# medvedevgroup/SibeliaZ

Measured on AMD Instinct MI355X. Metric: seed vertices/sec through BlocksFinder, higher is better.
Workload: dtype int32

## Files before the change

sibeliaz_amd/csrc/lcb_kernel.h:

```cpp
#ifndef LCB_KERNEL_H
#define LCB_KERNEL_H

#include <hip/hip_runtime.h>
#include <stdint.h>

#include "lcb_kernel_limits.h"

#define LCB_EMPTY_KEY INT32_MIN
#if defined(__HIP_DEVICE_COMPILE__)
#define LCB_NO_LOADS_IN_FLIGHT() __builtin_amdgcn_s_waitcnt(0x0F70)
#else
#define LCB_NO_LOADS_IN_FLIGHT() ((void)0)
#endif
#if defined(__HIP_DEVICE_COMPILE__)
#define LCB_GLOBAL_U32(p) ((const __attribute__((address_space(1))) uint32_t*)(p))
#else
#define LCB_GLOBAL_U32(p) (p)
#endif
#ifndef LCB_PROF_PUSH
#define LCB_PROF_PUSH 0
#endif

template <int MODE> struct LcbCfg;
template <> struct LcbCfg<0> { static constexpr uint32_t IC = 256, VC = 1024, BW = 256, PC = 0; static constexpr bool INST_LDS = true, IDX_LDS = true, WINDOW_WALK = true, RESOLVE = false; typedef uint16_t Idx; typedef uint32_t VLast; };
// ... 186 lines not shown
    uint8_t* fpSeg8;
    uint32_t* fpSeg32;
    uint32_t nFp;
    uint32_t fpSplit, fpShift;
    uint32_t instCap;
    int32_t* vKey;
    uint32_t* vCount;
    VLast* vLast;
    Idx* vTouched;
    uint32_t* vNClaimed;
    uint32_t* vTicket;
    uint32_t* vOvf;
    uint32_t* vRec;
    uint32_t* vItem;
    uint32_t voteCap, voteShift;
    uint32_t* scr;
    uint32_t* bloom;
    uint32_t bloomShift;
    uint32_t* mail;
    uint32_t* part;
    unsigned long long* mailWalk;
    int32_t* pKeys;
    uint32_t* pSlots;
    uint32_t pathCap, pathShift;
    unsigned long long* body;
    uint32_t bodyCap;
    uint4* best;
    uint32_t bestCap;
    uint32_t* ck;
    uint32_t ckN, ckInst, ckGood, ckPath;
    int32_t ckFlank;
    uint32_t nInst, nGood, cur, nPath, nRight, nLeft, nBest, status;
    int32_t rightFlank, leftFlank;
    uint32_t* dbg;
    const uint32_t* abort;
    uint32_t pfPush, pfVote, pfMaxProbe, pfMaxInst;
    uint64_t pfTVote, pfTPush, pfTScore;
    uint64_t pfTWalk, pfTWaitB, pfTReduce, pfTScan;
    uint64_t pfVoters, pfChunks, pfTouchSum;
    uint64_t cWalk, cOcc, cCompatCall, cCompatStep, cVote, cPush;
};

#ifndef LCB_TEST_FP_SLOT_DIV
#define LCB_TEST_FP_SLOT_DIV 1u
#endif
template <class ST>
__device__ __forceinline__ uint32_t lcb_fp_slot(const ST& S, uint32_t i)
{
    if (i < S.fpSplit) return i;
    const uint32_t f = i + S.fpShift;
    return f < S.instCap / LCB_TEST_FP_SLOT_DIV ? f : i;
}

template <class ST>
__device__ __forceinline__ void lcb_fp_set_seg(ST& S, uint32_t fs, uint32_t seg)
{
    if (ST::SEG) { if (LcbCfg<ST::MODE>::INST_LDS) S.fpSeg8[fs] = (uint8_t)seg; else S.fpSeg32[fs] = seg; }
}
template <class ST>
__device__ __forceinline__ uint32_t lcb_fp_get_seg(const ST& S, uint32_t fs)
{
    return ST::SEG ? (LcbCfg<ST::MODE>::INST_LDS ? (uint32_t)S.fpSeg8[fs] : S.fpSeg32[fs]) : 0u;
}

enum { LCB_F_FRONTG = 0, LCB_F_BACKG, LCB_F_FRONTPOS, LCB_F_BACKPOS, LCB_F_LO, LCB_F_HI, LCB_F_FLAGS, LCB_F_FRONTDIST, LCB_F_BACKDIST, LCB_F_COUNT };
template <class ST>
// ... 58 lines not shown
    const uint32_t wa = (uint32_t)(a >> 5), wb = (uint32_t)((b - 1) >> 5);
    const uint32_t ma = 0xFFFFFFFFu << ((uint32_t)a & 31), mb = 0xFFFFFFFFu >> (31 - ((uint32_t)(b - 1) & 31));
    if (wa == wb) return (lcb_uword(U, wa) & ma & mb) != 0;
    if (lcb_uword(U, wa) & ma) return true;
    for (uint32_t w = wa + 1; w < wb; w++)
        if (lcb_uword(U, w)) return true;
    return (lcb_uword(U, wb) & mb) != 0;
}

template <class F>
__device__ inline uint32_t lcb_range_walk_steps(const LcbUsed& used, F a, F b, bool up)
{
    uint32_t steps = 0;
    if (up) { for (F g = a; g < b; g++) { steps++; if (lcb_used_bit(used, g)) break; } }
    else { for (F g = b; g > a; g--) { steps++; if (lcb_used_bit(used, (F)(g - 1))) break; } }
    return steps;
}

__device__ __forceinline__ uint32_t lcb_bcast(uint32_t v, uint32_t src) { return (uint32_t)__shfl((int)v, (int)src); }

#define LCB_DPP_ADD64(v, ctrl, rowMask)                                                                             \
    do {                                                                                                            \
        const uint32_t lo_ = (uint32_t)__builtin_amdgcn_update_dpp(0, (int)(uint32_t)(v), ctrl, rowMask, 0xf, false); \
        const uint32_t hi_ = (uint32_t)__builtin_amdgcn_update_dpp(0, (int)(uint32_t)((v) >> 32), ctrl, rowMask, 0xf, false); \
        (v) += ((uint64_t)hi_ << 32) | lo_;                                                                         \
    } while (0)
__device__ __forceinline__ int64_t lcb_wave_sum(int64_t x)
{
    uint64_t v = (uint64_t)x;
    LCB_DPP_ADD64(v, 0x111, 0xf); LCB_DPP_ADD64(v, 0x112, 0xf); LCB_DPP_ADD64(v, 0x114, 0xf); LCB_DPP_ADD64(v, 0x118, 0xf);
    LCB_DPP_ADD64(v, 0x142, 0xa); LCB_DPP_ADD64(v, 0x143, 0xc);
    return (int64_t)(((uint64_t)lcb_rl((uint32_t)(v >> 32), 63) << 32) | lcb_rl((uint32_t)v, 63));
}

__device__ __forceinline__ uint32_t lcb_bloom1(int32_t vid, uint32_t sh) { return ((uint32_t)vid * 2654435761u) >> sh; }
__device__ __forceinline__ uint32_t lcb_bloom2(int32_t vid, uint32_t sh) { return ((uint32_t)vid * 0xC2B2AE35u + 0x27D4EB2Fu) >> sh; }

template <class ST>
__device__ __forceinline__ bool lcb_bloom_maybe(const ST& S, int32_t vid)
{
    const uint32_t a = lcb_bloom1(vid, S.bloomShift), b = lcb_bloom2(vid, S.bloomShift);
    return ((S.bloom[a >> 5] >> (a & 31)) & (S.bloom[b >> 5] >> (b & 31)) & 1u) != 0;
}

template <class ST>
__device__ inline bool lcb_path_probe(const ST& S, int32_t vid, uint32_t& probes)
{
    uint32_t h = lcb_hash(vid, S.pathShift);
    const uint32_t mask = S.pathCap - 1;
    uint32_t probe = 0;
    int32_t k = S.pKeys[h];
    while (k != vid && k != LCB_EMPTY_KEY && probe < S.pathCap) {
        h = (h + 1) & mask; probe++;
        k = S.pKeys[h];
    }
    probes = probe;
    return k == vid;
}

template <class ST>
__device__ __forceinline__ bool lcb_path_contains(const ST& S, int32_t vid)
{
    if (LcbCfg<ST::MODE>::BW && !lcb_bloom_maybe(S, vid)) return false;
    uint32_t probes;
    return lcb_path_probe(S, vid, probes);
}

template <class ST>
__device__ inline void lcb_path_insert(ST& S, int32_t vid)
{
    if ((S.nPath + 1) * 2 > S.pathCap) { S.status = LCB_ST_PATH_OVF; return; }
    uint32_t h = lcb_hash(vid, S.pathShift);
    const uint32_t mask = S.pathCap - 1;
    uint32_t probe = 0;
    while (S.pKeys[h] != LCB_EMPTY_KEY && probe < S.pathCap) { h = (h + 1) & mask; probe++; }
    if (probe == S.pathCap) { S.status = LCB_ST_PATH_OVF; return; }
    constexpr bool PL = LcbCfg<ST::MODE>::PC != 0;
    LCB_SYNC_IF(PL);
    if (S.lane == 0) {
        S.pKeys[h] = vid; S.pSlots[S.nPath] = h;
        if (LcbCfg<ST::MODE>::BW) {
            const uint32_t a = lcb_bloom1(vid, S.bloomShift), b = lcb_bloom2(vid, S.bloomShift);
            S.bloom[a >> 5] |= 1u << (a & 31);
            S.bloom[b >> 5] |= 1u << (b & 31);
        }
    }
    S.nPath++;
    LCB_SYNC_IF(PL);
}

template <class ST>
__device__ inline void lcb_path_clear(ST& S)
{
    constexpr uint32_t BW = LcbCfg<ST::MODE>::BW;
    for (uint32_t i = S.lane; i < S.nPath; i += 64) S.pKeys[S.pSlots[i]] = LCB_EMPTY_KEY;
    if (BW && S.nPath) for (uint32_t i = S.lane; i < (uint32_t)BW; i += 64) S.bloom[i] = 0;
    S.nPath = 0; S.nRight = 0; S.nLeft = 0; S.nInst = 0; S.nGood = 0; S.cur = 0; S.nTouch = 0;
    S.rightFlank = 0; S.leftFlank = 0;
    if (ST::SEG && S.lane <= LCB_MAX_SEG) S.segFirst[S.lane] = 0;
    LCB_WAVE_SYNC();
}

__device__ __forceinline__ uint32_t lcb_absdiff(uint32_t a, uint32_t b) { return a > b ? a - b : b - a; }

template <class ST>
__device__ __forceinline__ int64_t lcb_real_length(const ST& S, uint32_t i)
{
    return (int64_t)lcb_absdiff(S.iFrontPos[i], S.iBackPos[i]);
}

template <class ST>
__device__ inline void lcb_order_merge(ST& S, uint32_t m)
{
    const uint32_t n = S.nInst - m;
    const uint32_t c = S.cur, d = c ^ 1;
    const uint32_t* ck = S.ordKey + c * S.instCap; const typename ST::Idx* ci = S.ordIdx + c * S.instCap;
    uint32_t* dk = S.ordKey + d * S.instCap; typename ST::Idx* di = S.ordIdx + d * S.instCap;
    for (uint32_t i = S.lane; i < n; i += 64) {
        uint32_t cnt = 0;
        for (uint32_t r = 0; r < m; r++) cnt += (S.scr[r] <= i) ? 1u : 0u;
        dk[i + cnt] = ck[i];
        di[i + cnt] = ci[i];
    }
    if (S.lane < m) {
        const uint32_t at = S.scr[S.lane] + S.lane;
        dk[at] = S.scr[64 + S.lane];
        di[at] = (typename ST::Idx)S.scr[128 + S.lane];
    }
    if (ST::SEG && S.lane <= LCB_MAX_SEG) {
        uint32_t cnt = 0;
        for (uint32_t r = 0; r < m; r++) cnt += (S.scr[192 + r] < S.lane) ? 1u : 0u;
        S.segFirst[S.lane] += cnt;
    }
    S.cur = d;
    LCB_SYNC_IF(LcbCfg<ST::MODE>::IDX_LDS);
}

template <bool STATS, class ST>
__device__ inline void lcb_path_init(ST& S, int32_t vid, int32_t ch)
{
    const LcbTables& T = S.T;
    lcb_path_insert(S, vid);
    if (S.status) return;
    const uint32_t av = (uint32_t)(vid < 0 ? -vid : vid);
    typedef typename ST::Flat Flat;
    typedef typename ST::OccIdx OccIdx;
    const OccIdx o0 = lcb_rfl(lcb_occ_start<ST::SEG>(T, av)), o1 = lcb_rfl(lcb_occ_start<ST::SEG>(T, av + 1));
    for (OccIdx base = o0; base < o1; base += 64) {
        const OccIdx j = base + S.lane;
        bool ok = false;
        uint32_t g = 0, chr = 0, lo = 0, hi = 0, pos = 0;
        bool positive = false;
        if (j < o1) {
            if (STATS) S.cOcc++;
            const uint4 rec = T.occRec[j];
            g = rec.x; chr = rec.y; pos = rec.z;
            const uint2 lh = T.chrLoHi[chr & LCB_CHR_MASK];
            lo = lh.x; hi = lh.y;
            positive = ((int32_t)rec.w == vid);
            const Flat sb = lcb_seg_base(S, lcb_cw_seg(chr));
            ok = !lcb_it_used(S.U, sb, g, positive, lo) && (int32_t)lcb_it_char(T, (Flat)(sb + g), positive) == ch;
        }
        const unsigned long long m = __ballot(ok);
        const uint32_t cnt = (uint32_t)__popcll(m);
        if (S.nInst + cnt > S.instCap) { S.status = LCB_ST_INST_OVF; return; }
        if (ok) {
            const uint32_t i = S.nInst + (uint32_t)__popcll(m & ((1ull << S.lane) - 1));
            S.iFrontG[i] = g; S.iBackG[i] = g; S.iFrontPos[i] = pos; S.iBackPos[i] = pos;
            S.iFrontDist[i] = 0; S.iBackDist[i] = 0; S.iLo[i] = lo; S.iHi[i] = hi;
            S.iFlags[i] = (chr << LCB_FLAG_BITS) | (positive ? LCB_FLAG_POS : 0u);
            if (i >= S.nFp) { S.fpLo[i] = g; S.fpHi[i] = g; lcb_fp_set_seg(S, i, lcb_cw_seg(chr)); }
            S.ordKey[S.cur * S.instCap + i] = g;
            S.ordIdx[S.cur * S.instCap + i] = (typename ST::Idx)i;
            S.goodPos[i] = ST::NONE;
// ... 805 lines not shown
    return any;
}

template <class J> struct LcbEdgeT { uint32_t gIt, segIt; bool itPositive; int32_t idIt, idN; uint32_t posIt, posN; int32_t ech; J o0; uint32_t nOcc; };

#define LCB_ACT_NONE 0u
#define LCB_ACT_SKIP 1u
#define LCB_ACT_EXT_P 2u
#define LCB_ACT_EXT_X 3u
#define LCB_ACT_INSERT 4u

template <bool BACK, bool STATS, bool PROF, class ST>
__device__ inline bool lcb_push(ST& S, const LcbEdgeT<typename ST::OccIdx>& E, bool record, const uint4& rec0)
{
    const LcbTables& T = S.T;
    typedef typename ST::Flat Flat;
    typedef typename ST::OccIdx OccIdx;
    constexpr bool HOIST = !LcbCfg<ST::MODE>::INST_LDS;
    const uint64_t tq0 = (PROF && LCB_PROF_PUSH) ? wall_clock64() : 0;
    const int32_t vertex = E.itPositive ? E.idN : -E.idN;
    const int32_t otherVertex = E.itPositive ? E.idIt : -E.idIt;
    const OccIdx o0 = E.o0, o1 = E.o0 + E.nOcc;
    LcbOccT<Flat> occ = lcb_finish_occ(S, rec0, S.lane < E.nOcc);
    bool inPath = LcbCfg<ST::MODE>::BW ? lcb_bloom_maybe(S, vertex) : true;
    if (inPath) { uint32_t probes = 0; inPath = lcb_path_probe(S, vertex, probes); if (PROF && probes > S.pfMaxProbe) S.pfMaxProbe = probes; }
    if (inPath) return false;
    const uint32_t length = lcb_absdiff(E.posN, E.posIt);
    const int32_t ech = E.ech;
    const int64_t dist64 = BACK ? (int64_t)S.rightFlank + length : (int64_t)S.leftFlank - (int64_t)length;
    if (dist64 > INT32_MAX || dist64 < -(int64_t)INT32_MAX) { S.status = LCB_ST_DIST_OVF; return false; }
    const int32_t distance = (int32_t)dist64;
    lcb_path_insert(S, vertex);
    if (S.status) return false;

    const int64_t B = S.P.maxBranch;
    uint32_t nTouch = 0;
    if (PROF && LCB_PROF_PUSH) S.pfTWalk += wall_clock64() - tq0;
    for (OccIdx base = o0; base < o1; base += 64) {
        const uint64_t tq1 = (PROF && LCB_PROF_PUSH) ? wall_clock64() : 0;
        const OccIdx j = base + S.lane;
        const bool active = j < o1;
        const uint32_t n = S.nInst;
        const uint32_t* oKey = S.ordKey + S.cur * S.instCap;
        const typename ST::Idx* oIdx = S.ordIdx + S.cur * S.instCap;
        uint32_t g = 0, chr = 0, lo = 0, pos = 0, u = 0, cand = 0, act = LCB_ACT_NONE;
        uint32_t stCall = 0, stStep = 0;
        uint32_t lenBefore = 0, lenAfter = 0;
        bool positive = false, usedS = false, usesP = false;
        if (base != o0) occ = lcb_finish_occ(S, lcb_load_rec(T, j, active), active);
        if (active) {
            if (STATS) S.cOcc++;
            g = occ.rec.x; chr = occ.rec.y; pos = occ.rec.z;
            positive = ((int32_t)occ.rec.w == vertex);
            uint32_t a = 0, b = n;
            if (ST::SEG) { const uint32_t sg = lcb_cw_seg(chr); a = S.segFirst[sg]; b = S.segFirst[sg + 1]; }
            while (a < b) { const uint32_t mid = (a + b) >> 1; if (g < oKey[mid]) b = mid; else a = mid + 1; }
            u = a;
            uint32_t x = 0, p = 0, xFl = 0, pFl = 0;
            if (u < n) x = oIdx[u];
            if (u > 0) p = oIdx[u - 1];
            usesP = BACK ? positive : !positive;
            uint32_t hXF = 0, hXB = 0, hCG = 0, hCP = 0, hCO = 0;
            int32_t hCD = 0;
            if (HOIST) {
                const uint32_t c0 = usesP ? p : x;
                const bool hasC = usesP ? u > 0 : u < n;
                if (u < n) { xFl = S.iFlags[x]; hXF = S.iFrontG[x]; hXB = S.iBackG[x]; }
                if (u > 0) pFl = S.iFlags[p];
                if (hasC) {
                    hCG = BACK ? S.iBackG[c0] : S.iFrontG[c0]; hCP = BACK ? S.iBackPos[c0] : S.iFrontPos[c0];
                    hCD = BACK ? S.iBackDist[c0] : S.iFrontDist[c0]; hCO = BACK ? S.iFrontPos[c0] : S.iBackPos[c0];
                }
            } else {
                if (u < n) xFl = S.iFlags[x];
                if (u > 0) pFl = S.iFlags[p];
            }
            const bool hasX = u < n && (xFl >> LCB_FLAG_BITS) == chr;
            const bool hasP = u > 0 && (pFl >> LCB_FLAG_BITS) == chr;
            bool skip = false;
            if (hasX) {
                const uint32_t f = HOIST ? hXF : S.iFrontG[x], bk = HOIST ? hXB : S.iBackG[x];
                skip = g >= (f < bk ? f : bk) && g <= (f < bk ? bk : f);
            }
            if (skip) act = LCB_ACT_SKIP;
            else {
                const bool has = usesP ? hasP : hasX;
                bool compat = false;
                uint32_t cFl = 0;
                if (has) {
                    cand = usesP ? p : x;
                    cFl = usesP ? pFl : xFl;
                    if (STATS) stCall = 1;
                    const bool cpos = (cFl & LCB_FLAG_POS) != 0;
                    if (cpos == positive) {
                        const uint32_t cg = HOIST ? hCG : (BACK ? S.iBackG[cand] : S.iFrontG[cand]);
                        const uint32_t cp = HOIST ? hCP : (BACK ? S.iBackPos[cand] : S.iFrontPos[cand]);
                        const int32_t cd = HOIST ? hCD : (BACK ? S.iBackDist[cand] : S.iFrontDist[cand]);
                        lenBefore = lcb_absdiff(hCO, hCP); lenAfter = lcb_absdiff(hCO, pos);
                        const int64_t startPos = BACK ? cp : pos, endPos = BACK ? pos : cp;
                        const int64_t realDiff = positive ? endPos - startPos : startPos - endPos;
                        const int64_t ancestralDiff = BACK ? (int64_t)distance - cd : (int64_t)cd - distance;
                        const uint32_t ga = g < cg ? g : cg, gb = g < cg ? cg : g;
                        if (STATS) stStep = lcb_range_walk_steps(S.U, (Flat)(occ.sb + ga), (Flat)(occ.sb + gb), positive);
                        bool okDist = realDiff >= 0;
                        if (okDist && (realDiff > B || ancestralDiff > B)) {
                            const uint32_t gs = BACK ? cg : g, ge = BACK ? g : cg;
                            const bool adjacent = positive ? (ge == gs + 1) : (gs == ge + 1);
                            okDist = adjacent && (int32_t)lcb_it_char(T, (Flat)(occ.sb + gs), positive) == ech;
                            if (okDist && !BACK) {
                                const int32_t idE = T.posId[(Flat)(occ.sb + ge)];
                                okDist = (positive ? idE : -idE) == otherVertex;
                            }
                        }
                        compat = okDist && !lcb_range_any_used_c(S.U, occ, ga, gb);
                        if (cd == distance) compat = false;
                    }
                }
                lo = occ.lo;
                usedS = positive ? lcb_occ_bit(occ, g) : (g > lo ? lcb_occ_bit(occ, g - 1) : false);
                if (compat) {
                    const bool fin = (cFl & (BACK ? LCB_FLAG_BACKFIN : LCB_FLAG_FRONTFIN)) != 0;
                    act = fin ? LCB_ACT_NONE : (usesP ? LCB_ACT_EXT_P : LCB_ACT_EXT_X);
                } else act = usedS ? LCB_ACT_NONE : LCB_ACT_INSERT;
            }
        }
        const uint64_t tq2 = (PROF && LCB_PROF_PUSH) ? wall_clock64() : 0;
        if (PROF && LCB_PROF_PUSH) S.pfTWaitB += tq2 - tq1;
        const uint32_t uPrev = lcb_bcast(u, S.lane ? S.lane - 1 : 0);
        const uint32_t chrPrev = lcb_bcast(chr, S.lane ? S.lane - 1 : 0);
        const bool segStart = active && (S.lane == 0 || u != uPrev || chr != chrPrev);
        const unsigned long long startM = __ballot(segStart);
        const unsigned long long touchM = __ballot(active && (act == LCB_ACT_INSERT || act == LCB_ACT_EXT_P));
        const unsigned long long extXM = __ballot(active && act == LCB_ACT_EXT_X);
        if (active) {
            const unsigned long long below = (1ull << S.lane) - 1;
            const unsigned long long mineStart = startM & (below | (1ull << S.lane));
            const uint32_t s0 = 63u - (uint32_t)__clzll((long long)mineStart);
            const unsigned long long seg = below & ~((1ull << s0) - 1);
            if (extXM & seg) { act = LCB_ACT_SKIP; stCall = 0; stStep = 0; }
            else if (usesP && act != LCB_ACT_SKIP && (touchM & seg)) act = usedS ? LCB_ACT_NONE : LCB_ACT_INSERT;
        }
        if (STATS) {
            const unsigned long long finalTouchM = __ballot(active && (act == LCB_ACT_INSERT || act == LCB_ACT_EXT_P));
            const unsigned long long below = (1ull << S.lane) - 1;
            const unsigned long long mineStart = startM & (below | (1ull << S.lane));
            const uint32_t s0 = mineStart ? 63u - (uint32_t)__clzll((long long)mineStart) : 0u;
            const unsigned long long prior = active ? (finalTouchM & below & ~((1ull << s0) - 1)) : 0ull;
            const uint32_t t = prior ? 63u - (uint32_t)__clzll((long long)prior) : 0u;
            const uint32_t gT = lcb_bcast(g, t);
            const uint32_t posT = lcb_bcast(positive ? 1u : 0u, t);
            if (active && usesP && prior && !(extXM & below & ~((1ull << s0) - 1)) && act != LCB_ACT_SKIP) {
                stCall = 1;
                stStep = (posT != 0) == positive ? lcb_range_walk_steps(S.U, (Flat)(occ.sb + gT), (Flat)(occ.sb + g), positive) : 0u;
            }
            S.cCompatCall += stCall; S.cCompatStep += stStep;
        }
        const bool ins = active && act == LCB_ACT_INSERT;
        const bool ext = active && (act == LCB_ACT_EXT_P || act == LCB_ACT_EXT_X);
        bool becameGood = false;
        if (ext) {
            const int64_t before = HOIST ? (int64_t)lenBefore : lcb_real_length(S, cand);
            if (BACK) {
                S.iBackG[cand] = g; S.iBackPos[cand] = pos; S.iBackDist[cand] = distance;
                if (positive) S.ordKey[S.cur * S.instCap + u - 1] = g;
                if (usedS) S.iFlags[cand] |= LCB_FLAG_BACKFIN;
            } else {
                S.iFrontG[cand] = g; S.iFrontPos[cand] = pos; S.iFrontDist[cand] = distance;
                if (!positive) S.ordKey[S.cur * S.instCap + u - 1] = g;
                if (usedS) S.iFlags[cand] |= LCB_FLAG_FRONTFIN;
            }
            const uint32_t fs = lcb_fp_slot(S, cand);
            if (HOIST) { atomicMin(&S.fpLo[fs], g); atomicMax(&S.fpHi[fs], g); }
            else { if (g < S.fpLo[fs]) S.fpLo[fs] = g; if (g > S.fpHi[fs]) S.fpHi[fs] = g; }
            becameGood = before < (int64_t)S.P.minBlock && (HOIST ? (int64_t)lenAfter : lcb_real_length(S, cand)) >= (int64_t)S.P.minBlock;
        }
        if (ST::SEG) {
            bool clash = false;
            const unsigned long long im = __ballot(ins);
            if (ins) {
                const uint32_t i = S.nInst + (uint32_t)__popcll(im & ((1ull << S.lane) - 1));
                const uint32_t fs = lcb_fp_slot(S, i);
                clash = fs < S.nFp && lcb_fp_get_seg(S, fs) != lcb_cw_seg(chr);
            }
            if (__ballot(clash)) { S.status = LCB_ST_INST_OVF; return true; }
        }
        const unsigned long long insM = __ballot(ins);
        const unsigned long long extM = __ballot(ext);
        const unsigned long long goodM = __ballot(becameGood);
        const uint32_t m = (uint32_t)__popcll(insM);
        if (S.nInst + m > S.instCap) { S.status = LCB_ST_INST_OVF; return true; }
        if (becameGood) {
            const uint32_t at = S.nGood + (uint32_t)__popcll(goodM & ((1ull << S.lane) - 1));
            S.good[at] = (typename ST::Idx)cand; S.goodPos[cand] = (typename ST::Idx)at;
        }
        S.nGood += (uint32_t)__popcll(goodM);
        if (ext) S.touch[nTouch + (uint32_t)__popcll(extM & ((1ull << S.lane) - 1))] = (typename ST::Idx)cand;
        nTouch += (uint32_t)__popcll(extM);
        if (ins) {
            const uint32_t r = (uint32_t)__popcll(insM & ((1ull << S.lane) - 1));
            const uint32_t i = S.nInst + r;
            S.iFrontG[i] = g; S.iBackG[i] = g; S.iFrontPos[i] = pos; S.iBackPos[i] = pos;
            S.iFrontDist[i] = distance; S.iBackDist[i] = distance; S.iLo[i] = lo;
            S.iHi[i] = occ.hi;
            S.iFlags[i] = (chr << LCB_FLAG_BITS) | (positive ? LCB_FLAG_POS : 0u);
            {
                const uint32_t fs = lcb_fp_slot(S, i);
                if (fs >= S.nFp) { S.fpLo[fs] = g; S.fpHi[fs] = g; lcb_fp_set_seg(S, fs, lcb_cw_seg(chr)); }
#ifndef LCB_TEST_PLAIN_FP_READ
                else if (HOIST) { atomicMin(&S.fpLo[fs], g); atomicMax(&S.fpHi[fs], g); }
#endif
                else { if (g < S.fpLo[fs]) S.fpLo[fs] = g; if (g > S.fpHi[fs]) S.fpHi[fs] = g; }
            }
            S.scr[r] = u; S.scr[64 + r] = g; S.scr[128 + r] = i;
            if (ST::SEG) S.scr[192 + r] = lcb_cw_seg(chr);
            S.goodPos[i] = ST::NONE;
            S.touch[nTouch + r] = (typename ST::Idx)i;
        }
        nTouch += m;
        S.nInst += m;
        if (m) { const uint32_t top = lcb_fp_slot(S, S.nInst - 1) + 1; if (top > S.nFp) S.nFp = top; if (S.nInst > S.nFp) S.nFp = S.nInst; }
        LCB_SYNC_IF(LcbCfg<ST::MODE>::INST_LDS && LcbCfg<ST::MODE>::IDX_LDS);
        const uint64_t tq3 = (PROF && LCB_PROF_PUSH) ? wall_clock64() : 0;
        if (PROF && LCB_PROF_PUSH) S.pfTReduce += tq3 - tq2;
        if (m) lcb_order_merge(S, m);
        if (PROF && LCB_PROF_PUSH) S.pfTScan += wall_clock64() - tq3;
    }
    if (BACK) {
        if (record) {
            if (S.nRight >= S.bodyCap) { S.status = LCB_ST_PATH_OVF; return true; }
            if (S.lane == 0) S.body[S.nRight] = ((unsigned long long)(E.itPositive ? 1u : 0u) << 40) | ((unsigned long long)E.segIt << 32) | E.gIt;
        }
        S.nRight++;
        S.rightFlank = distance;
    } else {
        S.nLeft++;
        S.leftFlank = distance;
    }
    S.nTouch = nTouch;
    if (STATS && S.lane == 0) S.cPush++;
    if (PROF) { S.pfPush++; if (S.nInst > S.pfMaxInst) S.pfMaxInst = S.nInst; }
    return true;
}

template <class ST>
__device__ inline int64_t lcb_score(const ST& S)
{
    int64_t sum = 0;
    bool bad = false;
    for (uint32_t e = S.lane; e < S.nGood; e += 64) {
        const uint32_t i = S.good[e];
        const int64_t rightPenalty = (int64_t)S.rightFlank - S.iBackDist[i];
        const int64_t leftPenalty = -(int64_t)S.leftFlank + S.iFrontDist[i];
        if (leftPenalty >= S.P.maxFlank || rightPenalty >= S.P.maxFlank) bad = true;
        else sum += lcb_real_length(S, i) - (rightPenalty + leftPenalty) * (rightPenalty + leftPenalty);
    }
    const bool anyBad = __ballot(bad) != 0;
    if (anyBad) return -(int64_t)INT32_MAX;
    if (S.nGood == 0) return 0;
    return lcb_wave_sum(sum);
}

template <class ST>
__device__ inline void lcb_snapshot(ST& S)
{
    if (S.nGood > S.bestCap) { S.status = LCB_ST_BEST_OVF; return; }
    for (uint32_t e = S.lane; e < S.nGood; e += 64) {
        const uint32_t i = S.good[e];
        const uint32_t fl = S.iFlags[i];
        uint4 r;
        r.x = (fl >> LCB_FLAG_BITS) & LCB_CHR_MASK; r.y = S.iFrontG[i] - S.iLo[i]; r.z = S.iBackG[i] - S.iLo[i]; r.w = (fl & LCB_FLAG_POS);
        S.best[e] = r;
    }
    S.nBest = S.nGood;
}

#define LCB_CK_EVERY 32u
template <class ST>
__device__ inline void lcb_checkpoint(ST& S)
{
    const uint32_t n = S.nInst, cap = S.bestCap;
    if (n > cap) return;
    uint32_t* c = S.ck;
    const uint32_t* oKey = S.ordKey + S.cur * S.instCap;
    const typename ST::Idx* oIdx = S.ordIdx + S.cur * S.instCap;
    for (uint32_t i = S.lane; i < n; i += 64) {
        c[i] = S.iBackG[i]; c[cap + i] = S.iBackPos[i]; c[2 * cap + i] = (uint32_t)S.iBackDist[i]; c[3 * cap + i] = S.iFlags[i];
        c[4 * cap + i] = oKey[i]; c[5 * cap + i] = oIdx[i];
    }
    if (ST::SEG && S.lane <= LCB_MAX_SEG) c[6 * cap + S.lane] = S.segFirst[S.lane];
    S.ckN = S.nRight; S.ckInst = n; S.ckGood = S.nGood; S.ckPath = S.nPath; S.ckFlank = S.rightFlank;
}

template <class ST>
__device__ inline void lcb_restore_checkpoint(ST& S)
{
    LCB_WAVE_SYNC();
    for (uint32_t i = S.ckPath + S.lane; i < S.nPath; i += 64) S.pKeys[S.pSlots[i]] = LCB_EMPTY_KEY;
    for (uint32_t e = S.ckGood + S.lane; e < S.nGood; e += 64) S.goodPos[S.good[e]] = ST::NONE;
    const uint32_t n = S.ckInst, cap = S.bestCap;
    const uint32_t* c = S.ck;
    uint32_t* oKey = S.ordKey + S.cur * S.instCap;
    typename ST::Idx* oIdx = S.ordIdx + S.cur * S.instCap;
    for (uint32_t i = S.lane; i < n; i += 64) {
        S.iBackG[i] = c[i]; S.iBackPos[i] = c[cap + i]; S.iBackDist[i] = (int32_t)c[2 * cap + i]; S.iFlags[i] = c[3 * cap + i];
        oKey[i] = c[4 * cap + i]; oIdx[i] = (typename ST::Idx)c[5 * cap + i];
    }
    if (ST::SEG && S.lane <= LCB_MAX_SEG) S.segFirst[S.lane] = c[6 * cap + S.lane];
    S.nPath = S.ckPath; S.nInst = n; S.nGood = S.ckGood; S.nRight = S.ckN; S.nLeft = 0;
    S.rightFlank = S.ckFlank; S.leftFlank = 0; S.nTouch = 0;
    LCB_WAVE_SYNC();
}

template <class J> struct LcbEdgeBatchT { uint32_t gIt, segIt, itPos, posIt, posN, nOcc; J o0; int32_t idIt, idN, ech; };

template <bool FORWARD, class ST>
__device__ inline uint32_t lcb_batch_from_walk(const ST& S, uint32_t seg, uint32_t g, int dir, bool positive, uint32_t lo, uint32_t hi, int32_t next, LcbEdgeBatchT<typename ST::OccIdx>& b)
{
    const LcbTables& T = S.T;
    typedef typename ST::Flat Flat;
    const Flat sb = ST::SEG ? (Flat)lcb_rfl(S.segBase[seg]) : (Flat)0;
    const int64_t q0 = (int64_t)g + (int64_t)dir * (int64_t)S.lane, q1 = q0 + dir;
    const bool v0 = q0 >= (int64_t)lo && q0 < (int64_t)hi, v1 = q1 >= (int64_t)lo && q1 < (int64_t)hi;
    b.gIt = (uint32_t)q0; b.segIt = seg; b.itPos = positive ? 1u : 0u;
    b.idIt = 0; b.idN = 0; b.posIt = 0; b.posN = 0; b.ech = 0; b.o0 = 0; b.nOcc = 0;
    int32_t ch0 = 0, ch1 = 0;
    if (v0) { b.idIt = (T.posId + sb)[(uint32_t)q0]; b.posIt = (T.posPos + sb)[(uint32_t)q0]; ch0 = (int32_t)lcb_it_char(T, (Flat)(sb + (uint32_t)q0), positive); }
    if (v1) { b.idN = (T.posId + sb)[(uint32_t)q1]; b.posN = (T.posPos + sb)[(uint32_t)q1]; ch1 = (int32_t)lcb_it_char(T, (Flat)(sb + (uint32_t)q1), positive); }
    b.ech = FORWARD ? ch0 : ch1;
    const unsigned long long hit = __ballot(v1 && (positive ? b.idN : -b.idN) == next);
    const unsigned long long out = __ballot(!v1);
    const unsigned long long endM = hit | out;
    const uint32_t firstEnd = endM ? (uint32_t)__ffsll((long long)endM) - 1u : 64u;
    uint32_t n = 64;
    if (hit && (uint32_t)__ffsll((long long)hit) - 1u == firstEnd) n = firstEnd + 1;
    else if (firstEnd < 64) n = firstEnd;
    if (S.lane < n) {
        const uint32_t av = (uint32_t)(b.idN < 0 ? -b.idN : b.idN);
        b.o0 = lcb_occ_start<ST::SEG>(T, av); b.nOcc = (uint32_t)(lcb_occ_start<ST::SEG>(T, av + 1) - b.o0);
    }
    return n;
}

// ... 33 lines not shown
    const uint64_t tv0 = PROF ? wall_clock64() : 0;
    if (S.abort && lcb_rfl(__hip_atomic_load(S.abort, __ATOMIC_RELAXED, __HIP_MEMORY_SCOPE_AGENT)) != 0) { S.status = LCB_ST_ABORTED; return false; }
    const int32_t next = lcb_vote<STATS, PROF, NW>(S, FORWARD, FORWARD ? 2u : 1u, oi);
    LCB_MARK(S, 6, 2); LCB_MARK(S, 7, (uint32_t)next);
    if (S.status) return false;
    if (PROF) S.pfTVote += wall_clock64() - tv0;
    bool success = false;
    if (next != 0) {
        constexpr bool ONE = !LcbCfg<ST::MODE>::INST_LDS;
        const uint32_t f = ONE ? lcb_inst_fields(S, oi) : 0u;
        const uint32_t ofl = ONE ? lcb_rl(f, LCB_F_FLAGS) : lcb_rfl(S.iFlags[oi]);
        const bool positive = (ofl & LCB_FLAG_POS) != 0;
        const uint32_t oseg = ST::SEG ? lcb_fl_seg(ofl) : 0u;
        uint32_t g = ONE ? (FORWARD ? lcb_rl(f, LCB_F_BACKG) : lcb_rl(f, LCB_F_FRONTG)) : lcb_rfl(FORWARD ? S.iBackG[oi] : S.iFrontG[oi]);
        const int dir = (FORWARD == positive) ? 1 : -1;
        const uint32_t lo = ONE ? lcb_rl(f, LCB_F_LO) : lcb_rfl(S.iLo[oi]), hi = ONE ? lcb_rl(f, LCB_F_HI) : lcb_rfl(S.iHi[oi]);
        for (;;) {
            LcbEdgeBatchT<typename ST::OccIdx> bt;
            const uint32_t nE = lcb_batch_from_walk<FORWARD>(S, oseg, g, dir, positive, lo, hi, next, bt);
            if (nE == 0) break;
            uint4 rec = lcb_load_rec(T, lcb_rl(bt.o0, 0) + S.lane, S.lane < lcb_rl(bt.nOcc, 0));
            for (uint32_t l = 0; l < nE; l++) {
                const LcbEdgeT<typename ST::OccIdx> E = lcb_edge_of(bt, l);
                uint4 recN = uint4{0u, 0u, 0u, 0u};
                if (l + 1 < nE) recN = lcb_load_rec(T, lcb_rl(bt.o0, l + 1) + S.lane, S.lane < lcb_rl(bt.nOcc, l + 1));
                LCB_MARK(S, 6, 3); LCB_MARK(S, 8, E.gIt);
                const uint64_t tp0 = PROF ? wall_clock64() : 0;
                success = lcb_push<FORWARD, STATS, PROF>(S, E, true, rec);
                const uint64_t tp1 = PROF ? wall_clock64() : 0;
                if (PROF) S.pfTPush += tp1 - tp0;
                LCB_MARK(S, 6, 4);
                if (S.status) return false;
                if (success) {
                    nowScore = lcb_score(S);
                    if (nowScore > bestScore) {
                        bestScore = nowScore;
                        if (FORWARD) bestRightSize = S.nRight + 1;
                        if (!FORWARD && nowScore > 0) { lcb_snapshot(S); if (S.status) return false; }
                        if (FORWARD && !STATS && S.nRight >= S.ckN + LCB_CK_EVERY) lcb_checkpoint(S);
                    }
                    if (PROF) S.pfTScore += wall_clock64() - tp1;
                }
                rec = recN;
            }
            if (nE < 64 || (positive ? lcb_rl(bt.idN, 63) : -lcb_rl(bt.idN, 63)) == next) break;
            g = (uint32_t)((int64_t)g + 64 * dir);
        }
    }
    return success;
}

template <int MODE, bool STATS, bool PROF, int NW, class ST>
__device__ inline void lcb_process_seed(ST& S, int32_t vid, int32_t ch, int64_t& bestScoreOut)
{
    int64_t score = 0, bestScore = 0;
    S.nBest = 0; S.status = LCB_ST_OK; S.ckN = 0; S.endInst = 0; S.fpSplit = 0xFFFFFFFFu; S.fpShift = 0;
    LCB_MARK(S, 2, 1);
    lcb_path_init<STATS>(S, vid, ch);
    LCB_MARK(S, 2, 2); LCB_MARK(S, 3, S.nInst);
    const bool dead = !STATS && !S.status && S.nInst == 0;
    uint32_t bestRightSize = 1;
    const int64_t minRun = 2 * (int64_t)S.P.maxBranch;
    if (!S.status && !dead) {
        for (;;) {
            bool ret = true, positive = false;
            const int64_t prevLength = (int64_t)S.rightFlank - S.leftFlank;
            while ((ret = lcb_extend<true, STATS, PROF, NW>(S, bestRightSize, bestScore, score)) &&
                   ((int64_t)S.rightFlank - S.leftFlank) - prevLength <= minRun)
                positive = positive || (score > 0);
            if (!ret || !positive || S.status) break;
        }
// ... 122 lines not shown
    S.ck = (uint32_t*)(slot + L.ck); S.ckN = S.ckInst = S.ckGood = S.ckPath = 0; S.ckFlank = 0;
    uint32_t* instBase;
    uint32_t instStride;
    uint32_t *fpBase;
    if (INST_LDS) { instBase = sInst; instStride = IC; fpBase = sFp; }
    else { instBase = (uint32_t*)(slot + L.inst); instStride = W.instCap; fpBase = (uint32_t*)(slot + L.fp); }
    S.fpLo = fpBase; S.fpHi = fpBase + instStride;
    S.fpSeg8 = sFpSeg; S.fpSeg32 = INST_LDS ? nullptr : fpBase + 2 * instStride;
    if (IDX_LDS) {
        S.instCap = IC;
        S.ordKey = sOrdKey; S.ordIdx = sOrdIdx; S.good = sGood; S.goodPos = sGoodPos; S.touch = sTouch;
        S.vKey = sVKey; S.vCount = sVCount; S.vLast = sVLast; S.vTouched = sVTouched;
        S.voteCap = VC;
        for (uint32_t h = threadIdx.x; h < VC; h += 64 * NW) { sVKey[h] = LCB_EMPTY_KEY; sVCount[h] = 0; sVLast[h] = 0; }
    } else {
        S.instCap = W.instCap;
        S.ordKey = (uint32_t*)(slot + L.ordKey); S.ordIdx = (Idx*)(slot + L.ordIdx);
        S.good = (Idx*)(slot + L.good); S.goodPos = (Idx*)(slot + L.goodPos); S.touch = (Idx*)(slot + L.touch);
        S.vKey = (int32_t*)(slot + L.vKey); S.vCount = (uint32_t*)(slot + L.vCount);
        S.vLast = (VLast*)(slot + L.vLast); S.vTouched = (Idx*)(slot + L.vTouched);
        S.voteCap = W.voteCap;
    }
    S.bloom = sBloom;
    S.bloomShift = BW ? 32u - (uint32_t)__ffs((int)(BW * 32u)) + 1u : 0u;
    for (uint32_t h = threadIdx.x; h < BW; h += 64 * NW) sBloom[h] = 0;
    S.voteShift = 32u - (uint32_t)__ffs((int)S.voteCap) + 1u;
    S.iFrontG = instBase; S.iBackG = instBase + instStride;
    S.iFrontPos = instBase + 2 * instStride; S.iBackPos = instBase + 3 * instStride;
    S.iLo = instBase + 4 * instStride; S.iHi = instBase + 5 * instStride;
    S.iFlags = instBase + 6 * instStride;
    S.iFrontDist = (int32_t*)(instBase + 7 * instStride);
    S.iBackDist = (int32_t*)(instBase + 8 * instStride);
    S.scr = sScr; S.vNClaimed = &sMisc[0]; S.vOvf = &sMisc[1]; S.vTicket = &sMisc[2];
    S.mail = sMail; S.mailWalk = sMailWalk; S.part = sPart;
    if (RESOLVE) { S.vRec = sVRec; S.vItem = sVItem; } else { S.vRec = nullptr; S.vItem = nullptr; }
    const uint32_t waveId = lcb_rfl(threadIdx.x >> 6);
    S.dbg = (W.dbg && waveId == 0) ? W.dbg + 16u * blockIdx.x : nullptr;
    S.abort = W.abort;
    LCB_MARK(S, 0, 1);
    if (threadIdx.x == 0) { sMisc[0] = 0; sMisc[1] = 0; sMisc[2] = 0; sMail[LCB_MAIL_CMD] = 0; sMailWalk[0] = 0; }
    S.nInst = S.nGood = S.cur = S.nPath = S.nRight = S.nLeft = S.nBest = 0; S.status = 0; S.nTouch = S.nInit = 0;
    S.rightFlank = S.leftFlank = 0;
    S.cWalk = S.cOcc = S.cCompatCall = S.cCompatStep = S.cVote = S.cPush = 0;
    S.pfPush = S.pfVote = S.pfMaxProbe = S.pfMaxInst = 0; S.pfTVote = S.pfTPush = S.pfTScore = 0; S.nFp = 0;
    S.pfTWalk = S.pfTWaitB = S.pfTReduce = S.pfTScan = 0; S.pfVoters = S.pfChunks = S.pfTouchSum = 0;
    LCB_WAVE_SYNC();
    if (NW > 1) {
        __syncthreads();
        if (waveId != 0) {
            for (;;) {
                __syncthreads();
                if (lcb_rfl(S.mail[LCB_MAIL_CMD]) == LCB_CMD_EXIT) return;
                S.U.tab = sArgs.usedTab;
                const uint32_t flags = lcb_rfl(S.mail[LCB_MAIL_FLAGS]);
                S.nTouch = lcb_rfl(S.mail[LCB_MAIL_NTOUCH]);
                S.fpSplit = lcb_rfl(S.mail[LCB_MAIL_FPSPLIT]); S.fpShift = lcb_rfl(S.mail[LCB_MAIL_FPSHIFT]);
                S.cWalk = 0;
                if (RESOLVE && (flags & LCB_VF_RESOLVED)) lcb_vote_items<false>(S, (flags & LCB_VF_FORWARD) != 0, lcb_rfl(S.mail[LCB_MAIL_NITEMS]));
                else lcb_vote_walk<STATS>(S, (flags & LCB_VF_FORWARD) != 0, (flags & LCB_VF_TRYUSED) != 0, (flags & LCB_VF_USEGOOD) != 0, waveId, NW, (flags & LCB_VF_EXACT) != 0);
                if (STATS) {
                    const unsigned long long w = (unsigned long long)lcb_wave_sum((int64_t)S.cWalk);
                    if (S.lane == 0 && w) atomicAdd(S.mailWalk, w);
                }
                __syncthreads();
                if (flags & LCB_VF_SHARE) {
                    uint32_t nTouched = lcb_rfl(*S.vNClaimed);
                    const uint32_t claimCap = S.voteCap - (S.voteCap >> 2);
                    if (nTouched > claimCap) nTouched = claimCap;
// ... 129 lines not shown
```

Measured before the change: 953,400.

## Maintain block score incrementally and snapshot only touched instances backward

Adds an incremental score state (score, sum of penalties, bound, validity) that is updated algebraically on each path extension and each instance extension, so lcb_score can skip the full scan over all good instances while the flank stays within a bound. It also caches a known-bad instance so the bad verdict can be checked in constant time. Backward snapshots now rewrite only the touched instances when the previous snapshot was taken one step earlier. The trade is extra wave reductions and bookkeeping on every push, plus a risk of overflow or drift in the 32-bit delta arithmetic, which is guarded by fallbacks to the full rescan.

After: 948,700. About the same (-0.5%).

```diff
diff --git a/sibeliaz_amd/csrc/lcb_kernel.h b/sibeliaz_amd/csrc/lcb_kernel.h
--- a/sibeliaz_amd/csrc/lcb_kernel.h
+++ b/sibeliaz_amd/csrc/lcb_kernel.h
@@ -242,6 +242,10 @@
     int32_t ckFlank;
     uint32_t nInst, nGood, cur, nPath, nRight, nLeft, nBest, status;
     int32_t rightFlank, leftFlank;
+    int64_t scScore, scSumP;
+    int32_t scBound;
+    uint32_t scValid;
+    uint32_t bestAt;
     uint32_t* dbg;
     const uint32_t* abort;
     uint32_t pfPush, pfVote, pfMaxProbe, pfMaxInst;
@@ -366,6 +370,31 @@
     LCB_DPP_ADD64(v, 0x142, 0xa); LCB_DPP_ADD64(v, 0x143, 0xc);
     return (int64_t)(((uint64_t)lcb_rl((uint32_t)(v >> 32), 63) << 32) | lcb_rl((uint32_t)v, 63));
 }
+__device__ __forceinline__ int32_t lcb_wave_sum32(int32_t x)
+{
+    uint32_t v = (uint32_t)x;
+    v += (uint32_t)__builtin_amdgcn_update_dpp(0, (int)v, 0x111, 0xf, 0xf, false);
+    v += (uint32_t)__builtin_amdgcn_update_dpp(0, (int)v, 0x112, 0xf, 0xf, false);
+    v += (uint32_t)__builtin_amdgcn_update_dpp(0, (int)v, 0x114, 0xf, 0xf, false);
+    v += (uint32_t)__builtin_amdgcn_update_dpp(0, (int)v, 0x118, 0xf, 0xf, false);
+    v += (uint32_t)__builtin_amdgcn_update_dpp(0, (int)v, 0x142, 0xa, 0xf, false);
+    v += (uint32_t)__builtin_amdgcn_update_dpp(0, (int)v, 0x143, 0xc, 0xf, false);
+    return (int32_t)lcb_rl(v, 63);
+}
+
+#define LCB_SCORE_FAST_MAX_FLANK 1024
+#define LCB_SCORE_SCAN32_MAX_GOOD (1u << 20)
+#define LCB_SCORE_MAX_DLEN (1u << 24)
+#define LCB_BEST_STALE 0xFFFFFFFFu
+#define LCB_SCORE_INCR(ST, STATS) (!(STATS))
+enum { LCB_SC_STALE = 0, LCB_SC_VALID, LCB_SC_BAD };
+enum { LCB_SC_SCORE_FAST = 0, LCB_SC_SCORE_KNOWN_BAD, LCB_SC_SCORE_FULL, LCB_SC_SCORE_MISMATCH, LCB_SC_SNAP_TOUCHED, LCB_SC_SNAP_FULL, LCB_SC_SNAP_MISMATCH, LCB_SC_COUNT };
+#ifdef LCB_TEST_SCORE_EVENT
+void LCB_TEST_SCORE_EVENT(int what);
+#define LCB_SCORE_EVENT(S, what) do { if ((S).lane == 0) LCB_TEST_SCORE_EVENT(what); } while (0)
+#else
+#define LCB_SCORE_EVENT(S, what) ((void)0)
+#endif
 
 __device__ __forceinline__ uint32_t lcb_bloom1(int32_t vid, uint32_t sh) { return ((uint32_t)vid * 2654435761u) >> sh; }
 __device__ __forceinline__ uint32_t lcb_bloom2(int32_t vid, uint32_t sh) { return ((uint32_t)vid * 0xC2B2AE35u + 0x27D4EB2Fu) >> sh; }
@@ -431,6 +460,7 @@
     if (BW && S.nPath) for (uint32_t i = S.lane; i < (uint32_t)BW; i += 64) S.bloom[i] = 0;
     S.nPath = 0; S.nRight = 0; S.nLeft = 0; S.nInst = 0; S.nGood = 0; S.cur = 0; S.nTouch = 0;
     S.rightFlank = 0; S.leftFlank = 0;
+    S.scValid = LCB_SC_STALE; S.bestAt = LCB_BEST_STALE;
     if (ST::SEG && S.lane <= LCB_MAX_SEG) S.segFirst[S.lane] = 0;
     LCB_WAVE_SYNC();
 }
@@ -474,6 +504,7 @@
 __device__ inline void lcb_path_init(ST& S, int32_t vid, int32_t ch)
 {
     const LcbTables& T = S.T;
+    S.scValid = LCB_SC_STALE; S.bestAt = LCB_BEST_STALE;
     lcb_path_insert(S, vid);
     if (S.status) return;
     const uint32_t av = (uint32_t)(vid < 0 ? -vid : vid);
@@ -1345,6 +1376,14 @@
     const int32_t distance = (int32_t)dist64;
     lcb_path_insert(S, vertex);
     if (S.status) return false;
+    if (LCB_SCORE_INCR(ST, STATS) && S.scValid == LCB_SC_VALID) {
+        if (length >= (uint32_t)S.P.maxFlank) S.scValid = LCB_SC_STALE;
+        else {
+            const int64_t nl = (int64_t)S.nGood * length;
+            S.scScore -= 2 * (int64_t)length * S.scSumP + nl * length;
+            S.scSumP += nl;
+        }
+    }
 
     const int64_t B = S.P.maxBranch;
     uint32_t nTouch = 0;
@@ -1359,6 +1398,7 @@
         uint32_t g = 0, chr = 0, lo = 0, pos = 0, u = 0, cand = 0, act = LCB_ACT_NONE;
         uint32_t stCall = 0, stStep = 0;
         uint32_t lenBefore = 0, lenAfter = 0;
+        int32_t candDist = 0;
         bool positive = false, usedS = false, usesP = false;
         if (base != o0) occ = lcb_finish_occ(S, lcb_load_rec(T, j, active), active);
         if (active) {
@@ -1409,6 +1449,7 @@
                         const uint32_t cg = HOIST ? hCG : (BACK ? S.iBackG[cand] : S.iFrontG[cand]);
                         const uint32_t cp = HOIST ? hCP : (BACK ? S.iBackPos[cand] : S.iFrontPos[cand]);
                         const int32_t cd = HOIST ? hCD : (BACK ? S.iBackDist[cand] : S.iFrontDist[cand]);
+                        candDist = cd;
                         lenBefore = lcb_absdiff(hCO, hCP); lenAfter = lcb_absdiff(hCO, pos);
                         const int64_t startPos = BACK ? cp : pos, endPos = BACK ? pos : cp;
                         const int64_t realDiff = positive ? endPos - startPos : startPos - endPos;
@@ -1472,7 +1513,10 @@
         const bool ext = active && (act == LCB_ACT_EXT_P || act == LCB_ACT_EXT_X);
         bool becameGood = false;
         if (ext) {
-            const int64_t before = HOIST ? (int64_t)lenBefore : lcb_real_length(S, cand);
+            if (!HOIST) {
+                const uint32_t oth = BACK ? S.iFrontPos[cand] : S.iBackPos[cand];
+                lenBefore = lcb_absdiff(oth, BACK ? S.iBackPos[cand] : S.iFrontPos[cand]); lenAfter = lcb_absdiff(oth, pos);
+            }
             if (BACK) {
                 S.iBackG[cand] = g; S.iBackPos[cand] = pos; S.iBackDist[cand] = distance;
                 if (positive) S.ordKey[S.cur * S.instCap + u - 1] = g;
@@ -1485,7 +1529,7 @@
             const uint32_t fs = lcb_fp_slot(S, cand);
             if (HOIST) { atomicMin(&S.fpLo[fs], g); atomicMax(&S.fpHi[fs], g); }
             else { if (g < S.fpLo[fs]) S.fpLo[fs] = g; if (g > S.fpHi[fs]) S.fpHi[fs] = g; }
-            becameGood = before < (int64_t)S.P.minBlock && (HOIST ? (int64_t)lenAfter : lcb_real_length(S, cand)) >= (int64_t)S.P.minBlock;
+            becameGood = (int64_t)lenBefore < (int64_t)S.P.minBlock && (int64_t)lenAfter >= (int64_t)S.P.minBlock;
         }
         if (ST::SEG) {
             bool clash = false;
@@ -1509,6 +1553,25 @@
         S.nGood += (uint32_t)__popcll(goodM);
         if (ext) S.touch[nTouch + (uint32_t)__popcll(extM & ((1ull << S.lane) - 1))] = (typename ST::Idx)cand;
         nTouch += (uint32_t)__popcll(extM);
+        if (LCB_SCORE_INCR(ST, STATS) && S.scValid == LCB_SC_VALID) {
+            const bool rel = ext && (int64_t)lenAfter >= (int64_t)S.P.minBlock;
+            if (__ballot(rel)) {
+                int32_t dS = 0, dP = 0;
+                bool odd = false;
+                if (rel) {
+                    const uint32_t mf = (uint32_t)S.P.maxFlank;
+                    const int32_t od = BACK ? S.iFrontDist[cand] : S.iBackDist[cand];
+                    const uint32_t np = BACK ? (uint32_t)od - (uint32_t)S.leftFlank : (uint32_t)S.rightFlank - (uint32_t)od;
+                    const uint32_t r = BACK ? (uint32_t)distance - (uint32_t)candDist : (uint32_t)candDist - (uint32_t)distance;
+                    const uint32_t dl = becameGood ? lenAfter : lenAfter - lenBefore;
+                    odd = np >= mf || dl >= LCB_SCORE_MAX_DLEN || (!becameGood && r >= 2u * mf);
+                    if (becameGood) { dP = (int32_t)np; dS = (int32_t)(dl - np * np); }
+                    else { dP = -(int32_t)r; dS = (int32_t)(dl + r * (2u * np + r)); }
+                }
+                if (__ballot(odd)) S.scValid = LCB_SC_STALE;
+                else { S.scScore += lcb_wave_sum32(dS); S.scSumP += lcb_wave_sum32(dP); }
+            }
+        }
         if (ins) {
             const uint32_t r = (uint32_t)__popcll(insM & ((1ull << S.lane) - 1));
             const uint32_t i = S.nInst + r;
@@ -1555,36 +1618,113 @@
     return true;
 }
 
-template <class ST>
-__device__ inline int64_t lcb_score(const ST& S)
+template <bool FORWARD, class ST>
+__device__ inline int64_t lcb_score_scan(const ST& S, bool keep, int32_t& laneSumP, uint32_t& laneMaxPen, uint32_t& badInst)
 {
     int64_t sum = 0;
     bool bad = false;
+    uint32_t laneBad = 0;
+    laneSumP = 0; laneMaxPen = 0; badInst = 0xFFFFFFFFu;
     for (uint32_t e = S.lane; e < S.nGood; e += 64) {
         const uint32_t i = S.good[e];
         const int64_t rightPenalty = (int64_t)S.rightFlank - S.iBackDist[i];
         const int64_t leftPenalty = -(int64_t)S.leftFlank + S.iFrontDist[i];
-        if (leftPenalty >= S.P.maxFlank || rightPenalty >= S.P.maxFlank) bad = true;
-        else sum += lcb_real_length(S, i) - (rightPenalty + leftPenalty) * (rightPenalty + leftPenalty);
-    }
-    const bool anyBad = __ballot(bad) != 0;
-    if (anyBad) return -(int64_t)INT32_MAX;
+        if (leftPenalty >= S.P.maxFlank || rightPenalty >= S.P.maxFlank) { bad = true; laneBad = i; }
+        else {
+            sum += lcb_real_length(S, i) - (rightPenalty + leftPenalty) * (rightPenalty + leftPenalty);
+            if (keep) {
+                laneSumP += (int32_t)(rightPenalty + leftPenalty);
+                const uint32_t pen = (uint32_t)(FORWARD ? rightPenalty : leftPenalty);
+                if (pen > laneMaxPen) laneMaxPen = pen;
+            }
+        }
+    }
+    const unsigned long long badM = __ballot(bad);
+    if (badM) { badInst = lcb_rl(laneBad, (uint32_t)__ffsll((long long)badM) - 1u); return -(int64_t)INT32_MAX; }
     if (S.nGood == 0) return 0;
     return lcb_wave_sum(sum);
 }
 
+template <bool FORWARD, bool STATS, class ST>
+__device__ inline int64_t lcb_score(ST& S)
+{
+    bool fast = false;
+    int64_t fastScore = -(int64_t)INT32_MAX;
+    if (LCB_SCORE_INCR(ST, STATS) && S.scValid == LCB_SC_VALID) {
+        fast = (FORWARD ? (uint32_t)S.rightFlank - (uint32_t)S.scBound : (uint32_t)S.scBound - (uint32_t)S.leftFlank) < (uint32_t)S.P.maxFlank;
+        fastScore = S.scScore;
+    } else if (LCB_SCORE_INCR(ST, STATS) && S.scValid == LCB_SC_BAD) {
+        const uint32_t i = (uint32_t)S.scBound;
+        const int64_t rightPenalty = (int64_t)S.rightFlank - lcb_rfl(S.iBackDist[i]);
+        const int64_t leftPenalty = -(int64_t)S.leftFlank + lcb_rfl(S.iFrontDist[i]);
+        fast = leftPenalty >= S.P.maxFlank || rightPenalty >= S.P.maxFlank;
+    }
+#ifndef LCB_TEST_SCORE_EVENT
+    if (fast) return fastScore;
+#endif
+    const bool keep = LCB_SCORE_INCR(ST, STATS) && S.P.maxFlank >= 1 && S.P.maxFlank <= LCB_SCORE_FAST_MAX_FLANK && S.P.minBlock >= 1 && S.nGood < LCB_SCORE_SCAN32_MAX_GOOD;
+    int32_t laneSumP;
+    uint32_t laneMaxPen, badInst;
+    const int64_t score = lcb_score_scan<FORWARD>(S, keep, laneSumP, laneMaxPen, badInst);
+#ifdef LCB_TEST_SCORE_EVENT
+    LCB_SCORE_EVENT(S, fast ? (S.scValid == LCB_SC_BAD ? LCB_SC_SCORE_KNOWN_BAD : LCB_SC_SCORE_FAST) : LCB_SC_SCORE_FULL);
+    if (fast) {
+        if (fastScore != score) LCB_SCORE_EVENT(S, LCB_SC_SCORE_MISMATCH);
+        return fastScore;
+    }
+#endif
+    S.scValid = LCB_SC_STALE;
+    if (LCB_SCORE_INCR(ST, STATS) && badInst != 0xFFFFFFFFu) { S.scBound = (int32_t)badInst; S.scValid = LCB_SC_BAD; }
+    else if (keep) {
+        const uint32_t maxPen = lcb_wave_umax(laneMaxPen);
+        S.scScore = score;
+        S.scSumP = lcb_wave_sum32(laneSumP);
+        S.scBound = FORWARD ? (int32_t)((uint32_t)S.rightFlank - maxPen) : (int32_t)((uint32_t)S.leftFlank + maxPen);
+        S.scValid = LCB_SC_VALID;
+    }
+    return score;
+}
+
+template <class ST>
+__device__ __forceinline__ uint4 lcb_best_record(const ST& S, uint32_t i)
+{
+    const uint32_t fl = S.iFlags[i];
+    uint4 r;
+    r.x = (fl >> LCB_FLAG_BITS) & LCB_CHR_MASK; r.y = S.iFrontG[i] - S.iLo[i]; r.z = S.iBackG[i] - S.iLo[i]; r.w = (fl & LCB_FLAG_POS);
+    return r;
+}
+
 template <class ST>
 __device__ inline void lcb_snapshot(ST& S)
 {
     if (S.nGood > S.bestCap) { S.status = LCB_ST_BEST_OVF; return; }
+    for (uint32_t e = S.lane; e < S.nGood; e += 64) S.best[e] = lcb_best_record(S, S.good[e]);
+    S.nBest = S.nGood;
+    S.bestAt = S.nLeft;
+}
+
+template <class ST>
+__device__ inline void lcb_snapshot_backward(ST& S)
+{
+    if (S.bestAt + 1 != S.nLeft) { lcb_snapshot(S); LCB_SCORE_EVENT(S, LCB_SC_SNAP_FULL); return; }
+    if (S.nGood > S.bestCap) { S.status = LCB_ST_BEST_OVF; return; }
+    for (uint32_t t = S.lane; t < S.nTouch; t += 64) {
+        const uint32_t i = S.touch[t];
+        const typename ST::Idx e = S.goodPos[i];
+        if (e != ST::NONE) S.best[e] = lcb_best_record(S, i);
+    }
+    S.nBest = S.nGood;
+    S.bestAt = S.nLeft;
+#ifdef LCB_TEST_SCORE_EVENT
+    LCB_WAVE_SYNC();
+    bool differs = false;
     for (uint32_t e = S.lane; e < S.nGood; e += 64) {
-        const uint32_t i = S.good[e];
-        const uint32_t fl = S.iFlags[i];
-        uint4 r;
-        r.x = (fl >> LCB_FLAG_BITS) & LCB_CHR_MASK; r.y = S.iFrontG[i] - S.iLo[i]; r.z = S.iBackG[i] - S.iLo[i]; r.w = (fl & LCB_FLAG_POS);
-        S.best[e] = r;
-    }
-    S.nBest = S.nGood;
+        const uint4 a = S.best[e], b = lcb_best_record(S, S.good[e]);
+        differs = differs || a.x != b.x || a.y != b.y || a.z != b.z || a.w != b.w;
+    }
+    LCB_SCORE_EVENT(S, LCB_SC_SNAP_TOUCHED);
+    if (__ballot(differs)) LCB_SCORE_EVENT(S, LCB_SC_SNAP_MISMATCH);
+#endif
 }
 
 #define LCB_CK_EVERY 32u
@@ -1621,6 +1761,7 @@
     if (ST::SEG && S.lane <= LCB_MAX_SEG) S.segFirst[S.lane] = c[6 * cap + S.lane];
     S.nPath = S.ckPath; S.nInst = n; S.nGood = S.ckGood; S.nRight = S.ckN; S.nLeft = 0;
     S.rightFlank = S.ckFlank; S.leftFlank = 0; S.nTouch = 0;
+    S.scValid = LCB_SC_STALE; S.bestAt = LCB_BEST_STALE;
     LCB_WAVE_SYNC();
 }
 
@@ -1720,11 +1861,11 @@
                 LCB_MARK(S, 6, 4);
                 if (S.status) return false;
                 if (success) {
-                    nowScore = lcb_score(S);
+                    nowScore = lcb_score<FORWARD, STATS>(S);
                     if (nowScore > bestScore) {
                         bestScore = nowScore;
                         if (FORWARD) bestRightSize = S.nRight + 1;
-                        if (!FORWARD && nowScore > 0) { lcb_snapshot(S); if (S.status) return false; }
+                        if (!FORWARD && nowScore > 0) { lcb_snapshot_backward(S); if (S.status) return false; }
                         if (FORWARD && !STATS && S.nRight >= S.ckN + LCB_CK_EVERY) lcb_checkpoint(S);
                     }
                     if (PROF) S.pfTScore += wall_clock64() - tp1;
@@ -1913,8 +2054,7 @@
     S.iFrontDist = (int32_t*)(instBase + 7 * instStride);
     S.iBackDist = (int32_t*)(instBase + 8 * instStride);
     S.scr = sScr; S.vNClaimed = &sMisc[0]; S.vOvf = &sMisc[1]; S.vTicket = &sMisc[2];
-    S.mail = sMail; S.mailWalk = sMailWalk; S.part = sPart;
-    if (RESOLVE) { S.vRec = sVRec; S.vItem = sVItem; } else { S.vRec = nullptr; S.vItem = nullptr; }
+    S.mail = sMail; S.mailWalk = sMailWalk; S.part = sPart;    if (RESOLVE) { S.vRec = sVRec; S.vItem = sVItem; } else { S.vRec = nullptr; S.vItem = nullptr; }
     const uint32_t waveId = lcb_rfl(threadIdx.x >> 6);
     S.dbg = (W.dbg && waveId == 0) ? W.dbg + 16u * blockIdx.x : nullptr;
     S.abort = W.abort;
```
